# DPDK/grout

Hardware: AMD Instinct MI355X
Metric: Mpps IPv4 forward, 64B pkts, ~1M-route FIB (device-resident), 1/8 GPU (higher is better)
Workload: dtype u8/u32 integer

## Files before the change

grout_amd/csrc/fwd4_kernel.h:

```cpp
#pragma once

#include "../../include/grout_hip.h"

#include <stdint.h>

#define FWD4_STAT_SLOTS 32
#define FWD4_STAT_SHARDS 64
#define FWD4_MAX_ETH_TYPES 16

struct fwd4_edges {
	uint16_t eth_type_be[FWD4_MAX_ETH_TYPES];
	uint8_t eth_type_edge[FWD4_MAX_ETH_TYPES];
	uint8_t n_eth_types;
	uint8_t mode[GR_HIP_IFACE_MODE_COUNT];
	uint8_t in_nh[8];
	uint8_t out_nh[8];
	uint8_t out_iface[8];
	uint8_t iout_type[8];
	uint8_t in6_nh[8];
	uint8_t out6_nh[8];
	uint8_t out6_iface[8];
};

#define FWD4_RX_MAC_OK 0x01
// ... 110 lines not shown
	uint32_t out_stride;
	uint32_t readable;
	uint32_t nhf_lds;
	uint32_t nhf6_lds;
	const uint32_t *top6;
	uint32_t top6_lds;
	uint32_t chunk;
	uint32_t order;
	uint32_t spin_max;
	uint32_t *err;
	uint32_t wg0, wgs;
	uint32_t ptrs;
	uint32_t nat;
};

struct __attribute__((aligned(64))) fwd4_res_desc {
	uint64_t seq;
	uint64_t helper_seq[7];
	struct fwd4_params A;
};

struct fwd4_res_params {
	struct fwd4_res_desc *descs;
	uint64_t *done;
	uint64_t *exited;
	uint32_t *stop;
	uint64_t *wake;
	uint64_t *active;
	const uint32_t *taken;
	uint64_t lifetime;
// ... 14 lines not shown
```

grout_amd/csrc/fwd4_ring.hip:

```cpp
#include "fwd4_chain.h"

#define RING_GLDS_PER_TILE 6
#define RING_SPIN_MAX (1u << 24)
#define RING_NHF_LDS_MAX 2304

template <int WAVES_, int LOADERS_, int STORERS_, int SLOTS_, int AHEAD_>
struct ring_cfg {
	static constexpr uint32_t WAVES = WAVES_, LOADERS = LOADERS_, STORERS = STORERS_;
	static constexpr uint32_t COMPUTE = WAVES_ - LOADERS_ - STORERS_;
	static constexpr uint32_t SLOTS = SLOTS_, AHEAD = AHEAD_;
	static constexpr int VMCNT_AHEAD = RING_GLDS_PER_TILE * (AHEAD_ - 1);
	static_assert(COMPUTE >= 1 && SLOTS_ >= LOADERS_ * AHEAD_ && VMCNT_AHEAD <= 63, "ring geometry");
};

typedef ring_cfg<8, 1, 1, 8, 4> ring_cfg0;
typedef ring_cfg<8, 2, 1, 8, 3> ring_cfg1;
typedef ring_cfg<16, 2, 2, 16, 4> ring_cfg2;
typedef ring_cfg<12, 2, 1, 12, 4> ring_cfg3;
typedef ring_cfg<8, 1, 1, 8, 6> ring_cfg4;
typedef ring_cfg<16, 2, 2, 16, 6> ring_cfg5;
typedef ring_cfg<16, 3, 1, 20, 4> ring_cfg6;
typedef ring_cfg<16, 4, 2, 24, 3> ring_cfg7;
typedef ring_cfg<16, 2, 2, 16, 8> ring_cfg8;
typedef ring_cfg<14, 1, 1, 8, 8> ring_cfg9;
typedef ring_cfg<14, 2, 2, 8, 4> ring_cfg10;
typedef ring_cfg<12, 1, 1, 8, 8> ring_cfg11;
#define RING_NCFG 15

template <class C, bool PTRS>
struct ring_lds {
	uint8_t lines[C::SLOTS][64 * 64];
	u2v meta[C::SLOTS][64];
	uint64_t ptrs[PTRS ? C::SLOTS : 1][64];
	uint32_t ready[C::SLOTS], done[C::SLOTS], free_[C::SLOTS];
	uint32_t abort;
	uint32_t spin_max;
};

template <int N>
__device__ __forceinline__ void wait_vmcnt() {
	asm volatile("s_waitcnt vmcnt(%0)" ::"n"(N) : "memory");
}

__device__ __forceinline__ uint32_t lds_addr(const void *p) {
	return (uint32_t)(uintptr_t)(const __attribute__((address_space(3))) void *)p;
}

template <bool NT>
__device__ __forceinline__ void glds16(const void *gsrc, uint32_t lds_base) {
	uint32_t keep;
	if (NT)
// ... 11 lines not shown
template <bool NT>
__device__ __forceinline__ void glds4(const void *gsrc, uint32_t lds_base) {
	uint32_t keep;
	if (NT)
		asm volatile("s_mov_b32 %0, m0\n\ts_mov_b32 m0, %2\n\ts_nop 0\n\tglobal_load_lds_dword %1, off nt\n\ts_mov_b32 m0, %0"
			     : "=&s"(keep)
			     : "v"(gsrc), "s"(lds_base)
			     : "memory");
	else
		asm volatile("s_mov_b32 %0, m0\n\ts_mov_b32 m0, %2\n\ts_nop 0\n\tglobal_load_lds_dword %1, off\n\ts_mov_b32 m0, %0"
			     : "=&s"(keep)
			     : "v"(gsrc), "s"(lds_base)
			     : "memory");
}

__device__ __forceinline__ uint32_t flag_get(const uint32_t *f) {
	return __hip_atomic_load(f, __ATOMIC_RELAXED, __HIP_MEMORY_SCOPE_WORKGROUP);
}

__device__ __forceinline__ void flag_set(uint32_t *f, uint32_t v) {
	compiler_fence();
	__hip_atomic_store(f, v, __ATOMIC_RELAXED, __HIP_MEMORY_SCOPE_WORKGROUP);
}

template <class L_t>
__device__ __forceinline__ bool flag_wait(L_t &L, const uint32_t *f, uint32_t want) {
	const uint32_t lim = L.spin_max;
	for (uint32_t spin = 0;; spin++) {
		if ((int32_t)(flag_get(f) - want) >= 0)
			return true;
		if (flag_get(&L.abort))
			return false;
		if (spin >= lim) {
			flag_set(&L.abort, 1);
			return false;
		}
		__builtin_amdgcn_s_sleep(1);
	}
}

__device__ __forceinline__ uint32_t wg_id(const fwd4_params &A) {
	return A.wgs ? A.wg0 : blockIdx.x;
}
__device__ __forceinline__ uint32_t wg_count(const fwd4_params &A) {
	return A.wgs ? A.wgs : gridDim.x;
}

__device__ __forceinline__ uint32_t tile_of(const fwd4_params &A, uint32_t k) {
	const uint32_t b = wg_id(A), G = wg_count(A);
	if (A.order == 2) {
		const uint32_t x = b & 7, l = b >> 3, per = G >> 3;
		return x * A.chunk + l + k * per;
	}
	if (A.order == 3) {
		const uint32_t j = k / A.chunk;
// ... 18 lines not shown
	if (A.chunk)
		return b * A.chunk < n_tiles ? min(A.chunk, n_tiles - b * A.chunk) : 0;
	return b < n_tiles ? (n_tiles - 1 - b) / G + 1 : 0;
}

__device__ __forceinline__ uint64_t load_ptr(const fwd4_params &A, uint32_t t, uint32_t lane) {
	const uint32_t i = min(t * 64 + lane, A.n - 1);
	return gld(reinterpret_cast<const uint64_t *>(A.in) + i);
}

__device__ __forceinline__ uint64_t shfl64(uint64_t v, uint32_t src) {
	const uint32_t lo = __shfl((uint32_t)v, (int)src, 64), hi = __shfl((uint32_t)(v >> 32), (int)src, 64);
	return ((uint64_t)hi << 32) | lo;
}

template <class C, bool NT, bool PTRS, class LT>
__device__ void ring_loader(const fwd4_params &A, LT &L, uint32_t n_local, uint32_t j, uint32_t lane) {
	const uint32_t prow = lane >> 2;
	const uint32_t pchunk = (lane & 3) ^ ((lane >> 4) & 3);
	uint32_t pub = j;
	bool ok = true;
	uint64_t pnext = 0;
	if (PTRS && j < n_local)
		pnext = load_ptr(A, tile_of(A, j), lane);
	for (uint32_t k = j; k < n_local && ok; k += C::LOADERS) {
		const uint32_t s = k % C::SLOTS;
		if (k >= C::SLOTS && (int32_t)(flag_get(&L.free_[s]) - (k - C::SLOTS + 1)) < 0) {
			wait_vmcnt<0>();
			for (; pub < k; pub += C::LOADERS)
				flag_set(&L.ready[pub % C::SLOTS], pub + 1);
			ok = flag_wait(L, &L.free_[s], k - C::SLOTS + 1);
			if (!ok)
				break;
		}
		const uint32_t t = tile_of(A, k);
		const uint32_t base = t * 64, last = min(64u, A.n - base) - 1;
		uint64_t pk = 0;
		if (PTRS) {
			pk = pnext;
			if (k + C::LOADERS < n_local)
				pnext = load_ptr(A, tile_of(A, k + C::LOADERS), lane);
			if (k == j)
				wait_vmcnt<0>();
			else
				wait_vmcnt<RING_GLDS_PER_TILE>();
			L.ptrs[s][lane] = pk;
		}
		const uint32_t lb = lds_addr(L.lines[s]);
#pragma unroll
		for (uint32_t q = 0; q < 4; q++) {
			const uint32_t r = min(q * 16 + prow, last);
			const uint8_t *src = PTRS ? reinterpret_cast<const uint8_t *>(shfl64(pk, r))
						  : A.in + (size_t)(base + r) * A.in_stride;
			glds16<NT>(src + pchunk * 16, lb + q * 1024);
		}
		const uint32_t mb = lds_addr(L.meta[s]);
		const uint8_t *msrc = reinterpret_cast<const uint8_t *>(A.meta + base);
#pragma unroll
		for (uint32_t q = 0; q < 2; q++) {
			const uint32_t pkt = min(q * 32 + (lane >> 1), last);
			glds4<NT>(msrc + pkt * 8 + (lane & 1) * 4, mb + q * 256);
		}
		if (k - pub == (C::AHEAD - 1) * C::LOADERS) {
			wait_vmcnt<C::VMCNT_AHEAD>();
			flag_set(&L.ready[pub % C::SLOTS], pub + 1);
			pub += C::LOADERS;
		}
	}
	wait_vmcnt<0>();
	if (ok)
		for (; pub < n_local; pub += C::LOADERS)
			flag_set(&L.ready[pub % C::SLOTS], pub + 1);
}

template <class C, bool NT, bool PTRS, class LT>
__device__ void ring_storer(const fwd4_params &A, LT &L, uint32_t n_local, uint32_t j, uint32_t lane) {
	const uint32_t prow = lane >> 2, part = lane & 3;
	const uint32_t pslot = (part ^ ((lane >> 4) & 3)) << 4;
	const bool prefix = A.out_stride == GR_HIP_PREFIX;
	for (uint32_t k = j; k < n_local; k += C::STORERS) {
		const uint32_t s = k % C::SLOTS;
		if (!flag_wait(L, &L.done[s], k + 1))
			break;
		const uint32_t t = tile_of(A, k);
		const uint32_t base = t * 64, cnt = min(64u, A.n - base);
		u4v o[4];
#pragma unroll
		for (uint32_t q = 0; q < 4; q++)
			o[q] = *reinterpret_cast<const u4v *>(&L.lines[s][(q * 16 + prow) * 64 + pslot]);
		const u2v v = L.meta[s][lane];
		uint8_t *dst[4];
#pragma unroll
		for (uint32_t q = 0; q < 4; q++) {
			const uint32_t r = q * 16 + prow;
			dst[q] = PTRS && A.out == nullptr ? reinterpret_cast<uint8_t *>(L.ptrs[s][r])
							  : A.out + (size_t)(base + r) * A.out_stride;
		}
		asm volatile("s_waitcnt lgkmcnt(0)" ::: "memory");
		flag_set(&L.free_[s], k + 1);
// ... 29 lines not shown
		(const __attribute__((address_space(4))) uint32_t *)(((uint64_t)bhi << 32) | blo);
	uint32_t sv[SG];
#pragma unroll
	for (int i = 0; i < SG; i++)
		sv[i] = base[(uint32_t)__builtin_amdgcn_readlane(idx, i)];
	uint32_t v = 0, w = 0;
	if (want && lane >= (uint32_t)SG)
		v = gld(rx.tbl24 + idx);
#pragma unroll
	for (int i = 0; i < SG; i++)
		asm volatile("v_writelane_b32 %0, %1, %2" : "+v"(w) : "s"(sv[i]), "i"(i));
	ent = lane < (uint32_t)SG ? w : v;
	return want;
}

template <class C, bool STATS, bool PTRS, int SG = 0, class LT>
__device__ void ring_compute(const fwd4_params &A, const kctx &P, LT &L, stat_slot *slots,
			     const uint4 *nhf_lds, uint32_t n_local, uint32_t c, uint32_t lane) {
	for (uint32_t k = c; k < n_local; k += C::COMPUTE) {
		const uint32_t s = k % C::SLOTS;
		if (!flag_wait(L, &L.ready[s], k + 1))
			break;
		const uint32_t t = tile_of(A, k);
		const uint32_t base = t * 64, cnt = min(64u, A.n - base);
		const bool live = lane < cnt;
		uint8_t *R = L.lines[s];
		gr_hip_pkt_meta m = {0, 0, 0, 0};
		if (live) {
			const u2v pm = L.meta[s][lane];
			m.iface = pm.x & 0xffff;
			m.vlan_ck = pm.x >> 16;
			m.pkt_len = pm.y & 0xffff;
			m.rss = pm.y >> 16;
		}
		const uint32_t if0 = __builtin_amdgcn_readfirstlane(m.iface);
		rxv rx;
		if (__ballot(live && m.iface != if0) == 0)
			rx = load_rx_scalar(P, if0);
// ... 63 lines not shown
			c0.z = 0;
			lds_put(R, lane, 0, c0);
		}
		L.meta[s][lane] = u2v{r.edge | (r.domain << 8) | (r.iface << 16), r.nh};
		flag_set(&L.done[s], k + 1);
		if (STATS) {
			const uint32_t len = m.pkt_len;
			wave_count(slots, P, r.rx_if ? r.rx_if + 1 : 0, len);
			wave_count(slots, P, r.rx_par ? r.rx_par + 1 : 0, len);
			wave_count(slots, P, r.tx_if ? (r.tx_if | 0x10000u) + 1 : 0, len);
			wave_count(slots, P, r.tx_par ? (r.tx_par | 0x10000u) + 1 : 0, len);
		}
	}
}

#ifdef RING_TRACE
#define RING_TRACE_MAX 4096
__device__ uint64_t ring_trace[2 * RING_TRACE_MAX];
extern "C" int gr_fwd4_ring_trace(uint64_t *out, uint32_t n) {
	if (n > 2 * RING_TRACE_MAX)
		n = 2 * RING_TRACE_MAX;
	return hipMemcpyFromSymbol(out, HIP_SYMBOL(ring_trace), n * sizeof(uint64_t)) == hipSuccess ? 0 : -5;
}
#endif

template <class C, bool STATS, bool NT, bool PTRS = false, int SG = 0>
__global__ void __launch_bounds__(C::WAVES * 64) gr_fwd4_ring(const fwd4_params A) {
#ifdef RING_TRACE
	if (threadIdx.x == 0 && blockIdx.x < RING_TRACE_MAX)
		ring_trace[2 * blockIdx.x] = __builtin_amdgcn_s_memrealtime();
#endif
	__shared__ __attribute__((aligned(16))) ring_lds<C, PTRS> L;
	__shared__ stat_slot slots[FWD4_STAT_SLOTS];
	__shared__ fwd4_edges edges;
	extern __shared__ __attribute__((aligned(16))) uint4 nhf_lds[];
	const uint32_t tid = threadIdx.x, lane = tid & 63;
	const uint32_t wv = __builtin_amdgcn_readfirstlane(tid >> 6);
	const fwd4_tables *T = A.T;

	{
		const uint4 *src = reinterpret_cast<const uint4 *>(T->nhf) + 1;
		for (uint32_t i = tid; i < A.nhf_lds; i += C::WAVES * 64)
			nhf_lds[i] = gld4(src + i);
		const uint4 *src6 = reinterpret_cast<const uint4 *>(T->nhf6) + 1;
		for (uint32_t i = tid; i < A.nhf6_lds; i += C::WAVES * 64)
			nhf_lds[A.nhf_lds + i] = gld4(src6 + i);
		uint32_t *top6 = reinterpret_cast<uint32_t *>(nhf_lds + A.nhf_lds + A.nhf6_lds);
		for (uint32_t i = tid; i < A.top6_lds; i += C::WAVES * 64)
			top6[i] = gld(A.top6 + FWD4_TOP6_BASE + i);
	}
	for (uint32_t i = tid; i < sizeof(fwd4_edges); i += C::WAVES * 64)
		reinterpret_cast<uint8_t *>(&edges)[i] = reinterpret_cast<const uint8_t *>(&T->edges)[i];
	if (tid < C::SLOTS) {
		L.ready[tid] = 0;
		L.done[tid] = 0;
		L.free_[tid] = 0;
	}
	if (tid == 0) {
		L.abort = 0;
		L.spin_max = A.spin_max ? A.spin_max : RING_SPIN_MAX;
	}
	if (STATS && tid < FWD4_STAT_SLOTS) {
		slots[tid].key = 0;
		slots[tid].pkts = 0;
		slots[tid].bytes = 0;
	}
	__syncthreads();

	const uint32_t n_local = local_tiles(A);
	if (wv < C::LOADERS) {
		ring_loader<C, NT, PTRS>(A, L, n_local, wv, lane);
	} else if (wv < C::LOADERS + C::STORERS) {
		ring_storer<C, NT, PTRS>(A, L, n_local, wv - C::LOADERS, lane);
	} else {
		kctx P = make_kctx(A, &edges);
		P.nhf6_lds = (const __attribute__((address_space(3))) u4v *)(nhf_lds + A.nhf_lds);
		P.nhf6_n = A.nhf6_lds;
		P.top6 = A.top6;
		P.top6_lds = (const __attribute__((address_space(3))) uint32_t *)(nhf_lds + A.nhf_lds + A.nhf6_lds);
		P.top6_n = A.top6_lds;
		ring_compute<C, STATS, PTRS, SG>(A, P, L, slots, nhf_lds, n_local, wv - C::LOADERS - C::STORERS, lane);
	}

	__syncthreads();
	if (tid == 0 && L.abort && A.err != nullptr)
		__hip_atomic_store(A.err, 1u, __ATOMIC_RELAXED, __HIP_MEMORY_SCOPE_SYSTEM);
	if (STATS) {
		if (tid < FWD4_STAT_SLOTS && slots[tid].key != 0) {
			const uint32_t key = slots[tid].key - 1;
			shard_add(A.stats, T->max_ifaces, key >> 16, key & 0xffff, slots[tid].pkts, slots[tid].bytes);
		}
	}
#ifdef RING_TRACE
	__syncthreads();
	if (tid == 0 && blockIdx.x < RING_TRACE_MAX) {
		ring_trace[2 * blockIdx.x + 1] = __builtin_amdgcn_s_memrealtime();
	}
#endif
}

typedef ring_cfg2 ring_cfg_res;

__device__ __forceinline__ uint64_t sys_load64(const uint64_t *p) {
	return __hip_atomic_load(p, __ATOMIC_ACQUIRE, __HIP_MEMORY_SCOPE_SYSTEM);
}

__global__ void __launch_bounds__(ring_cfg_res::WAVES * 64) gr_fwd4_resident(const fwd4_res_params R) {
	typedef ring_cfg_res C;
	__shared__ __attribute__((aligned(16))) ring_lds<C, true> L;
	__shared__ __attribute__((aligned(16))) fwd4_params A;
	__shared__ fwd4_edges edges;
	__shared__ uint64_t seq_s;
	__shared__ uint32_t go;
	const uint32_t tid = threadIdx.x, lane = tid & 63;
	const uint32_t wv = __builtin_amdgcn_readfirstlane(tid >> 6);
	uint64_t *done = R.done + (size_t)blockIdx.x * R.stride;
	const fwd4_res_desc *ring = R.descs + (size_t)blockIdx.x * R.ndesc;
	uint64_t idle_since = __builtin_amdgcn_s_memrealtime();
	if (tid == 0) {
		seq_s = sys_load64(done) + 1;
		go = __hip_atomic_load(R.taken + blockIdx.x, __ATOMIC_RELAXED, __HIP_MEMORY_SCOPE_SYSTEM);
	}
	__syncthreads();
	if (go == 0) {
		if (tid == 0)
			__hip_atomic_store(R.exited + (size_t)blockIdx.x * R.stride, R.launch_id, __ATOMIC_RELEASE,
					   __HIP_MEMORY_SCOPE_SYSTEM);
		return;
	}
	const bool helper = go == 2;
// ... 56 lines not shown
			reinterpret_cast<uint8_t *>(&edges)[i] = reinterpret_cast<const uint8_t *>(&A.T->edges)[i];
		if (tid < C::SLOTS) {
			L.ready[tid] = 0;
			L.done[tid] = 0;
			L.free_[tid] = 0;
		}
		if (tid == 0) {
			L.abort = 0;
			L.spin_max = A.spin_max ? A.spin_max : RING_SPIN_MAX;
		}
		__syncthreads();
		const uint32_t n_local = local_tiles(A);
		const bool ptrs = A.ptrs != 0;
		if (wv < C::LOADERS) {
			if (ptrs)
				ring_loader<C, false, true>(A, L, n_local, wv, lane);
			else
				ring_loader<C, false, false>(A, L, n_local, wv, lane);
		} else if (wv < C::LOADERS + C::STORERS) {
			if (ptrs)
				ring_storer<C, false, true>(A, L, n_local, wv - C::LOADERS, lane);
			else
				ring_storer<C, false, false>(A, L, n_local, wv - C::LOADERS, lane);
		} else {
			const kctx P = make_kctx(A, &edges);
			if (ptrs)
				ring_compute<C, false, true>(A, P, L, nullptr, nullptr, n_local, wv - C::LOADERS - C::STORERS, lane);
			else
				ring_compute<C, false, false>(A, P, L, nullptr, nullptr, n_local, wv - C::LOADERS - C::STORERS, lane);
		}
		wait_vmcnt<0>();
		__syncthreads();
		if (tid == 0) {
			if (L.abort && A.err != nullptr)
				__hip_atomic_store(A.err, 1u, __ATOMIC_RELAXED, __HIP_MEMORY_SCOPE_SYSTEM);
			__hip_atomic_store(done, seq_s, __ATOMIC_RELEASE, __HIP_MEMORY_SCOPE_SYSTEM);
			seq_s++;
			idle_since = __builtin_amdgcn_s_memrealtime();
			__hip_atomic_store(R.active, idle_since, __ATOMIC_RELAXED, __HIP_MEMORY_SCOPE_AGENT);
		}
		__syncthreads();
	}
	if (tid == 0)
		__hip_atomic_store(R.exited + (size_t)blockIdx.x * R.stride, R.launch_id, __ATOMIC_RELEASE,
// ... 24 lines not shown
	const unsigned long long v = reset ? __hip_atomic_exchange(p, 0ull, __ATOMIC_RELAXED, __HIP_MEMORY_SCOPE_AGENT)
					   : __hip_atomic_fetch_add(p, 0ull, __ATOMIC_RELAXED, __HIP_MEMORY_SCOPE_AGENT);
	__hip_atomic_store(out + i, v, __ATOMIC_RELAXED, __HIP_MEMORY_SCOPE_SYSTEM);
}

extern "C" hipError_t gr_stats_collect_launch(void *d, void *out, uint32_t w, uint32_t pitch, uint32_t rows, int reset,
					      hipStream_t s) {
	const uint32_t n = w * 4 * rows;
	if (n == 0)
		return hipSuccess;
	hipLaunchKernelGGL(gr_stats_collect, dim3((n + 255) / 256), dim3(256), 0, s, static_cast<unsigned long long *>(d),
			   static_cast<unsigned long long *>(out), w, pitch, rows, reset);
	return hipGetLastError();
}

typedef void (*fwd4_rfn)(const fwd4_params);
struct ring_entry {
	fwd4_rfn fn[4];
	uint32_t threads;
};
#define RING_ENTRY_SG(C, SG) {{gr_fwd4_ring<C, false, false, false, SG>, gr_fwd4_ring<C, true, false, false, SG>, \
			 gr_fwd4_ring<C, false, true, false, SG>, gr_fwd4_ring<C, true, true, false, SG>}, C::WAVES * 64}
#define RING_ENTRY(C) RING_ENTRY_SG(C, 0)
static const ring_entry ring_kernels[RING_NCFG] = {
	RING_ENTRY(ring_cfg0), RING_ENTRY(ring_cfg1), RING_ENTRY(ring_cfg2),
	RING_ENTRY(ring_cfg3), RING_ENTRY(ring_cfg4), RING_ENTRY(ring_cfg5),
	RING_ENTRY(ring_cfg6), RING_ENTRY(ring_cfg7), RING_ENTRY(ring_cfg8),
	RING_ENTRY(ring_cfg9), RING_ENTRY(ring_cfg10), RING_ENTRY(ring_cfg11),
	RING_ENTRY_SG(ring_cfg2, 16), RING_ENTRY_SG(ring_cfg2, 32), RING_ENTRY_SG(ring_cfg2, 64),
};

#define RING_PTRS_CFG 2
typedef ring_cfg2 ring_cfg_ptrs;
static const ring_entry ring_ptrs_kernel = {
	{gr_fwd4_ring<ring_cfg_ptrs, false, false, true>, gr_fwd4_ring<ring_cfg_ptrs, true, false, true>,
	 gr_fwd4_ring<ring_cfg_ptrs, false, true, true>, gr_fwd4_ring<ring_cfg_ptrs, true, true, true>},
	ring_cfg_ptrs::WAVES * 64};

extern "C" hipError_t gr_fwd4_ring_launch(const fwd4_params *A, uint32_t grid, hipStream_t s, int variant, int cfg) {
	const ring_entry &e = (variant & FWD4_V_PTRS) ? ring_ptrs_kernel : ring_kernels[(unsigned)cfg % RING_NCFG];
	const size_t lds = (A->nhf_lds + A->nhf6_lds) * sizeof(fwd4_nhf) + A->top6_lds * sizeof(uint32_t);
	hipLaunchKernelGGL(e.fn[variant & 3], dim3(grid), dim3(e.threads), lds, s, *A);
	return hipGetLastError();
}

extern "C" uint32_t gr_fwd4_ring_nhf_max(void) {
	return RING_NHF_LDS_MAX;
}

extern "C" int gr_fwd4_ring_ncfg(void) {
	return RING_NCFG;
}

extern "C" int gr_fwd4_ring_occupancy(int variant, int cfg, uint32_t nhf_lds) {
	const ring_entry &e = (variant & FWD4_V_PTRS) ? ring_ptrs_kernel : ring_kernels[(unsigned)cfg % RING_NCFG];
	int b = 0;
	if (hipOccupancyMaxActiveBlocksPerMultiprocessor(&b, e.fn[variant & 3], (int)e.threads, nhf_lds * sizeof(fwd4_nhf))
// ... 7 lines not shown
```

grout_amd/csrc/gr_hip.cpp:

```cpp
#include <hip/hip_runtime.h>

#include "fib4.h"
#include "fib6.h"
#include "fwd4_kernel.h"
#include "gr_node_priv.h"

#include <algorithm>
#include <atomic>
#include <errno.h>
#include <map>
#include <mutex>
#include <shared_mutex>
#include <new>
#include <stdio.h>
#include <time.h>
#include <unistd.h>
#include <stdlib.h>
#include <string.h>
#include <vector>

extern "C" hipError_t gr_fwd4_ring_launch(const fwd4_params *A, uint32_t grid, hipStream_t s, int variant, int cfg);
extern "C" int gr_fwd4_ring_occupancy(int variant, int cfg, uint32_t nhf_lds);
extern "C" hipError_t gr_fwd4_resident_launch(const fwd4_res_params *R, uint32_t rings, hipStream_t s);
extern "C" hipError_t gr_stats_collect_launch(void *d, void *out, uint32_t w, uint32_t pitch, uint32_t rows, int reset,
					      hipStream_t s);
extern "C" uint32_t gr_fwd4_ring_nhf_max(void);
extern "C" int gr_fwd4_resident_occupancy(void);
extern "C" int gr_fwd4_ring_ncfg(void);
#define RING_WG_PER_CU 2


#define HCK(expr)                                                                                  \
	do {                                                                                       \
		hipError_t e__ = (expr);                                                           \
		if (e__ != hipSuccess) {                                                           \
			(void)hipGetLastError();                                                   \
			if (getenv("GR_HIP_TRACE_ERRORS"))                                         \
				fprintf(stderr, "gr_hip: %s:%d: %s: %s\n", __FILE__, __LINE__, #expr, \
					hipGetErrorString(e__));                                   \
			return e__ == hipErrorOutOfMemory ? -ENOMEM : -EIO;                        \
		}                                                                                  \
	} while (0)

namespace {
// ... 130 lines not shown
	bool own_stream;
	hipEvent_t ev0[N_TIMED], ev1[N_TIMED];
	uint64_t n_launch;
	uint64_t n_submit;
	bool always_timed;
	hipEvent_t quiesce;
	hipEvent_t retire;
	uint64_t seen_serial;
	hipEvent_t sync_ev;
	gr_hip_iface_stats *d_stats;
	host_slot hs[HOST_SLOTS];
	node_slot nw[GR_HIP_NODE_DEPTH];
	uint32_t nw_head, nw_count;
	uint8_t *d_pad;
	uint32_t *h_err, *d_err;
	std::vector<gr_hip_iface_stats> node_if;
	std::vector<gr_hip_iface_stats> kern_seen;
	gr_hip_iface_stats *snap = nullptr;
	void *snap_d = nullptr;
	uint32_t snap_cap = 0, snap_w = 0;
	gr_hip_iface_stats *rd = nullptr;
	void *rd_d = nullptr;
	uint32_t rd_cap = 0;
	hipEvent_t snap_ev = nullptr;
	bool snap_pending = false;
	uint64_t node_counted = 0, snap_counted = 0;
	uint8_t *pg_lines = nullptr, *pg_out = nullptr;
	gr_hip_pkt_meta *pg_meta = nullptr;
	gr_hip_verdict *pg_v = nullptr;
	uint32_t pg_cap = 0;
// ... 91 lines not shown
	uint32_t *d_snat_vals = nullptr;
	uint32_t snat_cap = 0;
	fwd4_edges edges;
	fwd4_tables *d_tables[2];
	std::vector<gr_hip_queue *> queues;
	int nt;
	int stats_on;
	int wg_per_cu;
	int fib_fmt;
	int ring_cfg;
	int host_direct;
	int node_ptrs;
	uint32_t stage_min_tiles;
	int tile_order;
	uint32_t tile_run;
	int alloc_contig;
	uint32_t spin_max;
	std::atomic<int> fail_appends{0};
	int untimed;
	uint32_t time_every;
	int stats_copy;
	int sync_check;
	std::atomic<int> host_path_last{-1};
	std::vector<host_range> hregs;
	int res_on;
	uint32_t res_rings;
	uint32_t res_w;
	uint32_t res_ms;
	uint32_t res_nap;
	uint32_t res_tiles;
// ... 472 lines not shown
		goto fail;
	if (hipMemsetAsync(c->d_adj, 0, sizeof(fwd4_adj) * ((size_t)max_nexthops + 1), c->ctl) != hipSuccess
	    || hipMemsetAsync(c->d_nhf, 0, sizeof(fwd4_nhf) * ((size_t)max_nexthops + 1), c->ctl) != hipSuccess
	    || hipMemsetAsync(c->d_nhf6, 0, sizeof(fwd4_nhf) * ((size_t)max_nexthops + 1), c->ctl) != hipSuccess
	    || hipMemsetAsync(c->d_adj6, 0, sizeof(fwd4_adj6) * ((size_t)max_nexthops + 1), c->ctl) != hipSuccess)
		goto fail;
	c->nt = FWD4_V_NT;
	c->stats_on = 1;
	c->wg_per_cu = 0;
	c->fib_fmt = FIB_FMT_24_W2;
	c->ring_cfg = 2;
	c->host_direct = 1;
	c->node_ptrs = 0;
	c->tile_order = 0;
	c->tile_run = 16;
	c->stage_min_tiles = 4;
	c->res_on = 0;
	c->res_rings = 256;
	c->res_w = 8;
	c->res_ms = 50;
	c->res_nap = 16;
	c->res_tiles = 8;
	c->spin_max = 0;
	c->untimed = 0;
	c->time_every = 1;
	c->alloc_contig = 1;
	for (int v = 0; v < 8; v++)
		c->occ_ring[v] = gr_fwd4_ring_occupancy(v, 0, 0);
	c->occ_n = 0;
	ret = -EIO;
// ... 1063 lines not shown
		hipEventCreate(&q->ev1[i]);
	}
	hipEventCreateWithFlags(&q->quiesce, hipEventDisableTiming);
	hipEventCreateWithFlags(&q->retire, hipEventDisableTiming);
	hipEventCreateWithFlags(&q->sync_ev, hipEventDisableTiming);
	for (node_slot &w : q->nw)
		hipEventCreateWithFlags(&w.done, hipEventDisableTiming);
	hipEventRecord(q->retire, q->s);
	if (hipHostMalloc(reinterpret_cast<void **>(&q->h_err), sizeof(uint32_t), hipHostMallocMapped) == hipSuccess) {
		*q->h_err = 0;
		if (hipHostGetDevicePointer(reinterpret_cast<void **>(&q->d_err), q->h_err, 0) != hipSuccess) {
			hipHostFree(q->h_err);
			q->h_err = q->d_err = nullptr;
		}
	}
	(void)hipGetLastError();
	size_t sb = sizeof(gr_hip_iface_stats) * FWD4_STAT_SHARDS * c->max_ifaces;
	if (hipMalloc(&q->d_stats, sb) != hipSuccess || hipMemsetAsync(q->d_stats, 0, sb, q->s) != hipSuccess) {
		(void)hipGetLastError();
		q->d_stats = nullptr;
	}
	try {
		q->node_if.assign(c->max_ifaces, gr_hip_iface_stats{0, 0, 0, 0});
		q->kern_seen.assign(c->max_ifaces, gr_hip_iface_stats{0, 0, 0, 0});
	} catch (...) {
		return -ENOMEM;
	}
	c->queues.push_back(q);
	*out = q;
	return 0;
// ... 36 lines not shown
		if (h.s)
			hipStreamDestroy(h.s);
		hipFree(h.in);
		hipFree(h.out);
		hipFree(h.meta);
		hipFree(h.v);
	}
	for (uint32_t i = 0; i < N_TIMED; i++) {
		hipEventDestroy(q->ev0[i]);
		hipEventDestroy(q->ev1[i]);
	}
	hipEventDestroy(q->quiesce);
	hipEventDestroy(q->retire);
	hipEventDestroy(q->sync_ev);
	hipFree(q->d_stats);
	if (q->snap_ev != nullptr)
		hipEventDestroy(q->snap_ev);
	hipHostFree(q->snap);
	hipHostFree(q->rd);
	hipHostFree(q->h_err);
	hipHostFree(q->pg_lines);
	hipHostFree(q->pg_out);
	hipHostFree(q->pg_meta);
	hipHostFree(q->pg_v);
	for (node_slot &w : q->nw) {
		hipEventDestroy(w.done);
		if (q->dead)
			continue;
		hipHostFree(w.lines);
		hipHostFree(w.out);
// ... 106 lines not shown
	uint32_t grid = (uint32_t)c->n_cu * per_cu;
	if (grid > tiles)
		grid = tiles;
	A.err = q->d_err;
	A.spin_max = c->spin_max;
	A.order = c->tile_order;
	A.chunk = 0;
	if (c->tile_order == 1)
		A.chunk = (tiles + grid - 1) / grid;
	if (c->tile_order == 2 && grid % 8 == 0)
		A.chunk = (tiles + 7) / 8;
	else if (c->tile_order == 2)
		A.order = 0;
	if (c->tile_order == 3)
		A.chunk = c->tile_run;
	if (timed && !q->always_timed) {
		const uint64_t k = q->n_submit++;
		timed = !c->untimed && (c->time_every <= 1 || k % c->time_every == 0);
	}
	if (timed)
		HCK(hipEventRecord(q->ev0[slot], s));
	HCK(gr_fwd4_ring_launch(&A, grid, s, variant, c->ring_cfg));
	if (timed) {
		HCK(hipEventRecord(q->ev1[slot], s));
		q->n_launch++;
	}
	return 0;
}

#define RES_NDESC 8
static_assert(GR_HIP_NODE_DEPTH < RES_NDESC, "a ring's batches in flight fit its descriptors");
#define RES_STRIDE 8
#define RES_TILES_PER_WG 8
#define RES_LEAVE_NS (500ull * 1000000ull)

static uint64_t res_word(const uint64_t *w, int ring) {
	return __atomic_load_n(w + (size_t)ring * RES_STRIDE, __ATOMIC_ACQUIRE);
// ... 455 lines not shown
		c->res_ms = (uint32_t)value;
	} else if (strcmp(key, "resident_launches") == 0) {
		return (int)c->res_launch;
	} else if (strcmp(key, "resident_ring_count") == 0) {
		return (int)c->res_rings;
	} else if (strcmp(key, "resident_busy") == 0) {
		return (int)c->res_busy.load();
	} else if (strcmp(key, "stage_min_tiles") == 0) {
		if (value < 0)
			return -EINVAL;
		c->stage_min_tiles = (uint32_t)value;
	} else if (strcmp(key, "tile_run") == 0) {
		if (value < 1 || value > 4096)
			return -EINVAL;
		c->tile_run = (uint32_t)value;
	} else if (strcmp(key, "host_direct") == 0) {
		c->host_direct = value != 0;
	} else if (strcmp(key, "fib_format_of") == 0) {
		if (value <= 0 || (uint32_t)value >= c->max_ifaces || c->vrfs[value].rib == nullptr
		    || !c->vrfs[value].uploaded())
			return -ENONET;
		return c->vrfs[value].pub().fmt;
	} else if (strcmp(key, "fib16") == 0) {
		c->fib_fmt = value ? FIB_FMT_16_8_8 : FIB_FMT_24;
	} else if (strcmp(key, "ring") == 0) {
		if (value < 0 || value >= gr_fwd4_ring_ncfg())
			return -EINVAL;
		c->ring_cfg = value;
	} else if (strncmp(key, "commit_us_", 10) == 0) {
		const char *k = key + 10;
// ... 1131 lines not shown
```

Before: 38620.

## Add dynamic tile claiming via global atomic counter for ring kernel tail balancing

The ring kernel now assigns most tiles statically, then leaves a tail share (default 32/256) that workgroups claim in runs of 8 tiles through a global atomic counter. The loader wave issues the atomic ahead of need and publishes run bases in LDS, and compute and storer waves read the tile id from LDS instead of recomputing it. The goal is to remove load imbalance and straggler workgroups at the end of each launch. The cost is an atomic round trip per run, extra LDS flags and end-of-stream handling, and a double-buffered counter that block 0 resets for the next launch.

```diff
diff --git a/grout_amd/csrc/fwd4_kernel.h b/grout_amd/csrc/fwd4_kernel.h
--- a/grout_amd/csrc/fwd4_kernel.h
+++ b/grout_amd/csrc/fwd4_kernel.h
@@ -148,6 +148,39 @@
 	uint32_t nat;
 };
 
+#define FWD4_CLAIM_SHARE_MAX 256u
+
+#ifdef __HIPCC__
+#define FWD4_HD __host__ __device__
+#else
+#define FWD4_HD
+#endif
+
+static inline FWD4_HD uint32_t fwd4_claim_n_static(uint32_t n_tiles, uint32_t G, uint32_t share) {
+	if (share > FWD4_CLAIM_SHARE_MAX)
+		share = FWD4_CLAIM_SHARE_MAX;
+	const uint32_t want = (uint32_t)(((uint64_t)n_tiles * share + FWD4_CLAIM_SHARE_MAX - 1) / FWD4_CLAIM_SHARE_MAX);
+	return G ? (n_tiles - want) / G : 0;
+}
+
+static inline FWD4_HD uint64_t fwd4_claim_run_base(uint32_t n_static, uint32_t G, uint32_t run, uint32_t g) {
+	return (uint64_t)n_static * G + (uint64_t)g * run;
+}
+
+static inline FWD4_HD uint32_t fwd4_claim_run_len(uint32_t n_tiles, uint64_t base, uint32_t run) {
+	if (base >= n_tiles)
+		return 0;
+	const uint32_t left = n_tiles - (uint32_t)base;
+	return left < run ? left : run;
+}
+
+struct fwd4_claim {
+	uint32_t *ctr;
+	uint32_t *ctr_next;
+	uint32_t n_static;
+	uint32_t run;
+};
+
 struct __attribute__((aligned(64))) fwd4_res_desc {
 	uint64_t seq;
 	uint64_t helper_seq[7];
diff --git a/grout_amd/csrc/fwd4_ring.hip b/grout_amd/csrc/fwd4_ring.hip
--- a/grout_amd/csrc/fwd4_ring.hip
+++ b/grout_amd/csrc/fwd4_ring.hip
@@ -3,6 +3,7 @@
 #define RING_GLDS_PER_TILE 6
 #define RING_SPIN_MAX (1u << 24)
 #define RING_NHF_LDS_MAX 2304
+#define RING_CLAIM_NR 64
 
 template <int WAVES_, int LOADERS_, int STORERS_, int SLOTS_, int AHEAD_>
 struct ring_cfg {
@@ -11,6 +12,7 @@
 	static constexpr uint32_t SLOTS = SLOTS_, AHEAD = AHEAD_;
 	static constexpr int VMCNT_AHEAD = RING_GLDS_PER_TILE * (AHEAD_ - 1);
 	static_assert(COMPUTE >= 1 && SLOTS_ >= LOADERS_ * AHEAD_ && VMCNT_AHEAD <= 63, "ring geometry");
+	static_assert(SLOTS_ + (AHEAD_ + 1) * LOADERS_ + 2 <= RING_CLAIM_NR, "claimed runs in LDS");
 };
 
 typedef ring_cfg<8, 1, 1, 8, 4> ring_cfg0;
@@ -35,6 +37,10 @@
 	uint32_t ready[C::SLOTS], done[C::SLOTS], free_[C::SLOTS];
 	uint32_t abort;
 	uint32_t spin_max;
+	uint32_t tile[C::SLOTS];
+	uint32_t run_base[RING_CLAIM_NR];
+	uint32_t runs;
+	uint32_t end;
 };
 
 template <int N>
@@ -76,6 +82,16 @@
 			     : "memory");
 }
 
+#ifdef RING_TRACE
+#define RING_TRACE_MAX 4096
+__device__ uint64_t ring_trace[4 * RING_TRACE_MAX];
+extern "C" int gr_fwd4_ring_trace(uint64_t *out, uint32_t n) {
+	if (n > 4 * RING_TRACE_MAX)
+		n = 4 * RING_TRACE_MAX;
+	return hipMemcpyFromSymbol(out, HIP_SYMBOL(ring_trace), n * sizeof(uint64_t)) == hipSuccess ? 0 : -5;
+}
+#endif
+
 __device__ __forceinline__ uint32_t flag_get(const uint32_t *f) {
 	return __hip_atomic_load(f, __ATOMIC_RELAXED, __HIP_MEMORY_SCOPE_WORKGROUP);
 }
@@ -101,6 +117,92 @@
 	}
 }
 
+template <class L_t>
+__device__ __forceinline__ int flag_wait_k(L_t &L, const uint32_t *f, uint32_t want, uint32_t k) {
+	const uint32_t lim = L.spin_max;
+	for (uint32_t spin = 0;; spin++) {
+		if ((int32_t)(flag_get(f) - want) >= 0)
+			return 1;
+		if (flag_get(&L.abort))
+			return 0;
+		const uint32_t e = flag_get(&L.end);
+		if (e != 0 && k >= e - 1)
+			return 2;
+		if (spin >= lim) {
+			flag_set(&L.abort, 1);
+			return 0;
+		}
+		__builtin_amdgcn_s_sleep(1);
+	}
+}
+
+__device__ __forceinline__ uint32_t claim_box() {
+	uint32_t box;
+	asm volatile("v_mov_b32 %0, 0" : "=v"(box));
+	return box;
+}
+
+__device__ __forceinline__ void claim_issue(uint32_t *ctr, uint32_t box) {
+	uint64_t keep;
+	asm volatile("s_mov_b64 %0, exec\n\ts_mov_b64 exec, 1\n\tglobal_atomic_add %1, %2, %3, off sc0\n\ts_mov_b64 exec, %0"
+		     : "=&s"(keep)
+		     : "v"(box), "v"(ctr), "v"(1u)
+		     : "memory");
+}
+
+template <int N>
+__device__ __forceinline__ uint32_t claim_read(uint32_t box) {
+	uint32_t g;
+	asm volatile("s_waitcnt vmcnt(%2)\n\tv_readfirstlane_b32 %0, %1" : "=s"(g) : "v"(box), "n"(N) : "memory");
+	return g;
+}
+
+struct claim_state {
+	uint32_t n_claim;
+	uint32_t since;
+	bool pending, ended;
+};
+
+template <int N, class LT>
+__device__ __forceinline__ void claim_take(const fwd4_params &A, const fwd4_claim &Q, LT &L, claim_state &cs, uint32_t box,
+					   uint32_t &n_known) {
+	const uint32_t g = claim_read<N>(box);
+	const uint32_t n_tiles = (A.n + 63) >> 6;
+	const uint64_t base = fwd4_claim_run_base(Q.n_static, gridDim.x, Q.run, g);
+	const uint32_t len = fwd4_claim_run_len(n_tiles, base, Q.run);
+	cs.pending = false;
+	if (len != 0)
+		L.run_base[cs.n_claim % RING_CLAIM_NR] = (uint32_t)base;
+	n_known += len;
+	if (len < Q.run) {
+		cs.ended = true;
+		flag_set(&L.end, n_known + 1);
+	}
+	cs.n_claim++;
+	flag_set(&L.runs, cs.n_claim);
+}
+
+template <class C, class LT>
+__device__ __forceinline__ void claim_step(const fwd4_params &A, const fwd4_claim &Q, LT &L, claim_state &cs, uint32_t box,
+					   uint32_t &n_known, uint32_t k) {
+	while (!cs.ended) {
+		if (cs.pending) {
+			if (cs.since < C::AHEAD - 1) {
+				if (k < n_known)
+					break;
+				wait_vmcnt<0>();
+			}
+			claim_take<C::VMCNT_AHEAD>(A, Q, L, cs, box, n_known);
+		} else {
+			if (k + C::AHEAD * C::LOADERS < n_known)
+				break;
+			claim_issue(Q.ctr, box);
+			cs.pending = true;
+			cs.since = 0;
+		}
+	}
+}
+
 __device__ __forceinline__ uint32_t wg_id(const fwd4_params &A) {
 	return A.wgs ? A.wg0 : blockIdx.x;
 }
@@ -149,8 +251,9 @@
 	return ((uint64_t)hi << 32) | lo;
 }
 
-template <class C, bool NT, bool PTRS, class LT>
-__device__ void ring_loader(const fwd4_params &A, LT &L, uint32_t n_local, uint32_t j, uint32_t lane) {
+template <class C, bool NT, bool PTRS, bool CLAIM, class LT>
+__device__ void ring_loader(const fwd4_params &A, const fwd4_claim &Q, LT &L, uint32_t n_local, uint32_t j, uint32_t lane) {
+	static_assert(!(CLAIM && PTRS), "frame-pointer launches keep the static order");
 	const uint32_t prow = lane >> 2;
 	const uint32_t pchunk = (lane & 3) ^ ((lane >> 4) & 3);
 	uint32_t pub = j;
@@ -158,7 +261,34 @@
 	uint64_t pnext = 0;
 	if (PTRS && j < n_local)
 		pnext = load_ptr(A, tile_of(A, j), lane);
-	for (uint32_t k = j; k < n_local && ok; k += C::LOADERS) {
+	const bool dyn = CLAIM && Q.ctr != nullptr;
+	claim_state cs = {0, 0, false, !dyn};
+	const uint32_t box = CLAIM ? claim_box() : 0;
+	uint32_t k = j;
+	for (; ok; k += C::LOADERS) {
+		uint32_t t = 0;
+		if (CLAIM && dyn && j == 0)
+			claim_step<C>(A, Q, L, cs, box, n_local, k);
+		if (CLAIM && dyn && k >= Q.n_static) {
+			const uint32_t i = (k - Q.n_static) / Q.run;
+			if (j != 0 && (int32_t)(flag_get(&L.runs) - (i + 1)) < 0) {
+				wait_vmcnt<0>();
+				for (; pub < k; pub += C::LOADERS)
+					flag_set(&L.ready[pub % C::SLOTS], pub + 1);
+				if (flag_wait_k(L, &L.runs, i + 1, k) == 0) {
+					ok = false;
+					break;
+				}
+			}
+			const uint32_t e = flag_get(&L.end);
+			if (e != 0 && k >= e - 1)
+				break;
+			t = __builtin_amdgcn_readfirstlane(L.run_base[i % RING_CLAIM_NR]) + (k - Q.n_static) % Q.run;
+		} else {
+			if (k >= n_local && cs.ended)
+				break;
+			t = tile_of(A, k);
+		}
 		const uint32_t s = k % C::SLOTS;
 		if (k >= C::SLOTS && (int32_t)(flag_get(&L.free_[s]) - (k - C::SLOTS + 1)) < 0) {
 			wait_vmcnt<0>();
@@ -168,8 +298,13 @@
 			if (!ok)
 				break;
 		}
-		const uint32_t t = tile_of(A, k);
 		const uint32_t base = t * 64, last = min(64u, A.n - base) - 1;
+		if (CLAIM)
+			L.tile[s] = t;
+#ifdef RING_TRACE
+		if (k == 0 && lane == 0 && blockIdx.x < RING_TRACE_MAX)
+			ring_trace[4 * blockIdx.x + 2] = __builtin_amdgcn_s_memrealtime();
+#endif
 		uint64_t pk = 0;
 		if (PTRS) {
 			pk = pnext;
@@ -196,6 +331,7 @@
 			const uint32_t pkt = min(q * 32 + (lane >> 1), last);
 			glds4<NT>(msrc + pkt * 8 + (lane & 1) * 4, mb + q * 256);
 		}
+		cs.since++;
 		if (k - pub == (C::AHEAD - 1) * C::LOADERS) {
 			wait_vmcnt<C::VMCNT_AHEAD>();
 			flag_set(&L.ready[pub % C::SLOTS], pub + 1);
@@ -204,20 +340,24 @@
 	}
 	wait_vmcnt<0>();
 	if (ok)
-		for (; pub < n_local; pub += C::LOADERS)
+		for (; pub < k; pub += C::LOADERS)
 			flag_set(&L.ready[pub % C::SLOTS], pub + 1);
-}
-
-template <class C, bool NT, bool PTRS, class LT>
+#ifdef RING_TRACE
+	if (CLAIM && j == 0 && lane == 0 && blockIdx.x < RING_TRACE_MAX)
+		ring_trace[4 * blockIdx.x + 3] = cs.n_claim;
+#endif
+}
+
+template <class C, bool NT, bool PTRS, bool CLAIM, class LT>
 __device__ void ring_storer(const fwd4_params &A, LT &L, uint32_t n_local, uint32_t j, uint32_t lane) {
 	const uint32_t prow = lane >> 2, part = lane & 3;
 	const uint32_t pslot = (part ^ ((lane >> 4) & 3)) << 4;
 	const bool prefix = A.out_stride == GR_HIP_PREFIX;
-	for (uint32_t k = j; k < n_local; k += C::STORERS) {
+	for (uint32_t k = j; CLAIM || k < n_local; k += C::STORERS) {
 		const uint32_t s = k % C::SLOTS;
-		if (!flag_wait(L, &L.done[s], k + 1))
+		if (CLAIM ? flag_wait_k(L, &L.done[s], k + 1, k) != 1 : !flag_wait(L, &L.done[s], k + 1))
 			break;
-		const uint32_t t = tile_of(A, k);
+		const uint32_t t = CLAIM ? __builtin_amdgcn_readfirstlane(L.tile[s]) : tile_of(A, k);
 		const uint32_t base = t * 64, cnt = min(64u, A.n - base);
 		u4v o[4];
 #pragma unroll
@@ -277,14 +417,14 @@
 	return want;
 }
 
-template <class C, bool STATS, bool PTRS, int SG = 0, class LT>
+template <class C, bool STATS, bool PTRS, bool CLAIM, int SG = 0, class LT>
 __device__ void ring_compute(const fwd4_params &A, const kctx &P, LT &L, stat_slot *slots,
 			     const uint4 *nhf_lds, uint32_t n_local, uint32_t c, uint32_t lane) {
-	for (uint32_t k = c; k < n_local; k += C::COMPUTE) {
+	for (uint32_t k = c; CLAIM || k < n_local; k += C::COMPUTE) {
 		const uint32_t s = k % C::SLOTS;
-		if (!flag_wait(L, &L.ready[s], k + 1))
+		if (CLAIM ? flag_wait_k(L, &L.ready[s], k + 1, k) != 1 : !flag_wait(L, &L.ready[s], k + 1))
 			break;
-		const uint32_t t = tile_of(A, k);
+		const uint32_t t = CLAIM ? __builtin_amdgcn_readfirstlane(L.tile[s]) : tile_of(A, k);
 		const uint32_t base = t * 64, cnt = min(64u, A.n - base);
 		const bool live = lane < cnt;
 		uint8_t *R = L.lines[s];
@@ -378,21 +518,14 @@
 	}
 }
 
+template <class C, bool STATS, bool NT, bool PTRS = false, int SG = 0>
+__global__ void __launch_bounds__(C::WAVES * 64) gr_fwd4_ring(const fwd4_params A, const fwd4_claim Q) {
+	constexpr bool CLAIM = !PTRS;
 #ifdef RING_TRACE
-#define RING_TRACE_MAX 4096
-__device__ uint64_t ring_trace[2 * RING_TRACE_MAX];
-extern "C" int gr_fwd4_ring_trace(uint64_t *out, uint32_t n) {
-	if (n > 2 * RING_TRACE_MAX)
-		n = 2 * RING_TRACE_MAX;
-	return hipMemcpyFromSymbol(out, HIP_SYMBOL(ring_trace), n * sizeof(uint64_t)) == hipSuccess ? 0 : -5;
-}
-#endif
-
-template <class C, bool STATS, bool NT, bool PTRS = false, int SG = 0>
-__global__ void __launch_bounds__(C::WAVES * 64) gr_fwd4_ring(const fwd4_params A) {
-#ifdef RING_TRACE
-	if (threadIdx.x == 0 && blockIdx.x < RING_TRACE_MAX)
-		ring_trace[2 * blockIdx.x] = __builtin_amdgcn_s_memrealtime();
+	if (threadIdx.x == 0 && blockIdx.x < RING_TRACE_MAX) {
+		ring_trace[4 * blockIdx.x] = __builtin_amdgcn_s_memrealtime();
+		ring_trace[4 * blockIdx.x + 3] = 0;
+	}
 #endif
 	__shared__ __attribute__((aligned(16))) ring_lds<C, PTRS> L;
 	__shared__ stat_slot slots[FWD4_STAT_SLOTS];
@@ -420,9 +553,13 @@
 		L.done[tid] = 0;
 		L.free_[tid] = 0;
 	}
+	const bool dyn = CLAIM && Q.ctr != nullptr;
+	const uint32_t n_local = dyn ? Q.n_static : local_tiles(A);
 	if (tid == 0) {
 		L.abort = 0;
 		L.spin_max = A.spin_max ? A.spin_max : RING_SPIN_MAX;
+		L.runs = 0;
+		L.end = dyn ? 0 : n_local + 1;
 	}
 	if (STATS && tid < FWD4_STAT_SLOTS) {
 		slots[tid].key = 0;
@@ -431,11 +568,10 @@
 	}
 	__syncthreads();
 
-	const uint32_t n_local = local_tiles(A);
 	if (wv < C::LOADERS) {
-		ring_loader<C, NT, PTRS>(A, L, n_local, wv, lane);
+		ring_loader<C, NT, PTRS, CLAIM>(A, Q, L, n_local, wv, lane);
 	} else if (wv < C::LOADERS + C::STORERS) {
-		ring_storer<C, NT, PTRS>(A, L, n_local, wv - C::LOADERS, lane);
+		ring_storer<C, NT, PTRS, CLAIM>(A, L, n_local, wv - C::LOADERS, lane);
 	} else {
 		kctx P = make_kctx(A, &edges);
 		P.nhf6_lds = (const __attribute__((address_space(3))) u4v *)(nhf_lds + A.nhf_lds);
@@ -443,12 +579,14 @@
 		P.top6 = A.top6;
 		P.top6_lds = (const __attribute__((address_space(3))) uint32_t *)(nhf_lds + A.nhf_lds + A.nhf6_lds);
 		P.top6_n = A.top6_lds;
-		ring_compute<C, STATS, PTRS, SG>(A, P, L, slots, nhf_lds, n_local, wv - C::LOADERS - C::STORERS, lane);
+		ring_compute<C, STATS, PTRS, CLAIM, SG>(A, P, L, slots, nhf_lds, n_local, wv - C::LOADERS - C::STORERS, lane);
 	}
 
 	__syncthreads();
 	if (tid == 0 && L.abort && A.err != nullptr)
 		__hip_atomic_store(A.err, 1u, __ATOMIC_RELAXED, __HIP_MEMORY_SCOPE_SYSTEM);
+	if (CLAIM && tid == 0 && blockIdx.x == 0 && Q.ctr_next != nullptr)
+		__hip_atomic_store(Q.ctr_next, 0u, __ATOMIC_RELAXED, __HIP_MEMORY_SCOPE_AGENT);
 	if (STATS) {
 		if (tid < FWD4_STAT_SLOTS && slots[tid].key != 0) {
 			const uint32_t key = slots[tid].key - 1;
@@ -457,9 +595,8 @@
 	}
 #ifdef RING_TRACE
 	__syncthreads();
-	if (tid == 0 && blockIdx.x < RING_TRACE_MAX) {
-		ring_trace[2 * blockIdx.x + 1] = __builtin_amdgcn_s_memrealtime();
-	}
+	if (tid == 0 && blockIdx.x < RING_TRACE_MAX)
+		ring_trace[4 * blockIdx.x + 1] = __builtin_amdgcn_s_memrealtime();
 #endif
 }
 
@@ -478,6 +615,7 @@
 	__shared__ uint32_t go;
 	const uint32_t tid = threadIdx.x, lane = tid & 63;
 	const uint32_t wv = __builtin_amdgcn_readfirstlane(tid >> 6);
+	const fwd4_claim Q0 = {nullptr, nullptr, 0, 0};
 	uint64_t *done = R.done + (size_t)blockIdx.x * R.stride;
 	const fwd4_res_desc *ring = R.descs + (size_t)blockIdx.x * R.ndesc;
 	uint64_t idle_since = __builtin_amdgcn_s_memrealtime();
@@ -564,20 +702,20 @@
 		const bool ptrs = A.ptrs != 0;
 		if (wv < C::LOADERS) {
 			if (ptrs)
-				ring_loader<C, false, true>(A, L, n_local, wv, lane);
+				ring_loader<C, false, true, false>(A, Q0, L, n_local, wv, lane);
 			else
-				ring_loader<C, false, false>(A, L, n_local, wv, lane);
+				ring_loader<C, false, false, false>(A, Q0, L, n_local, wv, lane);
 		} else if (wv < C::LOADERS + C::STORERS) {
 			if (ptrs)
-				ring_storer<C, false, true>(A, L, n_local, wv - C::LOADERS, lane);
+				ring_storer<C, false, true, false>(A, L, n_local, wv - C::LOADERS, lane);
 			else
-				ring_storer<C, false, false>(A, L, n_local, wv - C::LOADERS, lane);
+				ring_storer<C, false, false, false>(A, L, n_local, wv - C::LOADERS, lane);
 		} else {
 			const kctx P = make_kctx(A, &edges);
 			if (ptrs)
-				ring_compute<C, false, true>(A, P, L, nullptr, nullptr, n_local, wv - C::LOADERS - C::STORERS, lane);
+				ring_compute<C, false, true, false>(A, P, L, nullptr, nullptr, n_local, wv - C::LOADERS - C::STORERS, lane);
 			else
-				ring_compute<C, false, false>(A, P, L, nullptr, nullptr, n_local, wv - C::LOADERS - C::STORERS, lane);
+				ring_compute<C, false, false, false>(A, P, L, nullptr, nullptr, n_local, wv - C::LOADERS - C::STORERS, lane);
 		}
 		wait_vmcnt<0>();
 		__syncthreads();
@@ -632,7 +770,7 @@
 	return hipGetLastError();
 }
 
-typedef void (*fwd4_rfn)(const fwd4_params);
+typedef void (*fwd4_rfn)(const fwd4_params, const fwd4_claim);
 struct ring_entry {
 	fwd4_rfn fn[4];
 	uint32_t threads;
@@ -655,10 +793,11 @@
 	 gr_fwd4_ring<ring_cfg_ptrs, false, true, true>, gr_fwd4_ring<ring_cfg_ptrs, true, true, true>},
 	ring_cfg_ptrs::WAVES * 64};
 
-extern "C" hipError_t gr_fwd4_ring_launch(const fwd4_params *A, uint32_t grid, hipStream_t s, int variant, int cfg) {
+extern "C" hipError_t gr_fwd4_ring_launch(const fwd4_params *A, const fwd4_claim *Q, uint32_t grid, hipStream_t s, int variant,
+					  int cfg) {
 	const ring_entry &e = (variant & FWD4_V_PTRS) ? ring_ptrs_kernel : ring_kernels[(unsigned)cfg % RING_NCFG];
 	const size_t lds = (A->nhf_lds + A->nhf6_lds) * sizeof(fwd4_nhf) + A->top6_lds * sizeof(uint32_t);
-	hipLaunchKernelGGL(e.fn[variant & 3], dim3(grid), dim3(e.threads), lds, s, *A);
+	hipLaunchKernelGGL(e.fn[variant & 3], dim3(grid), dim3(e.threads), lds, s, *A, *Q);
 	return hipGetLastError();
 }
 
diff --git a/grout_amd/csrc/gr_hip.cpp b/grout_amd/csrc/gr_hip.cpp
--- a/grout_amd/csrc/gr_hip.cpp
+++ b/grout_amd/csrc/gr_hip.cpp
@@ -19,7 +19,8 @@
 #include <string.h>
 #include <vector>
 
-extern "C" hipError_t gr_fwd4_ring_launch(const fwd4_params *A, uint32_t grid, hipStream_t s, int variant, int cfg);
+extern "C" hipError_t gr_fwd4_ring_launch(const fwd4_params *A, const fwd4_claim *Q, uint32_t grid, hipStream_t s, int variant,
+						  int cfg);
 extern "C" int gr_fwd4_ring_occupancy(int variant, int cfg, uint32_t nhf_lds);
 extern "C" hipError_t gr_fwd4_resident_launch(const fwd4_res_params *R, uint32_t rings, hipStream_t s);
 extern "C" hipError_t gr_stats_collect_launch(void *d, void *out, uint32_t w, uint32_t pitch, uint32_t rows, int reset,
@@ -28,6 +29,32 @@
 extern "C" int gr_fwd4_resident_occupancy(void);
 extern "C" int gr_fwd4_ring_ncfg(void);
 #define RING_WG_PER_CU 2
+#define CLAIM_SHARE_DEFAULT 32
+#define CLAIM_RUN_DEFAULT 8
+#define CLAIM_MIN_TILES_DEFAULT 4096
+#define CLAIM_WORD_STRIDE 32
+
+extern "C" uint32_t gr_fwd4_claim_n_static(uint32_t n_tiles, uint32_t grid, uint32_t share) {
+	return fwd4_claim_n_static(n_tiles, grid, share);
+}
+extern "C" uint32_t gr_fwd4_claim_run(uint32_t n_tiles, uint32_t grid, uint32_t n_static, uint32_t run, uint32_t g,
+				      uint64_t *base) {
+	const uint64_t b = fwd4_claim_run_base(n_static, grid, run, g);
+	if (base != nullptr)
+		*base = b;
+	return fwd4_claim_run_len(n_tiles, b, run);
+}
+extern "C" uint32_t gr_fwd4_claim_runs(uint32_t n_tiles, uint32_t grid, uint32_t n_static, uint32_t run, uint64_t *base,
+				       uint32_t *len, uint32_t max) {
+	uint32_t first_empty = max;
+	for (uint32_t g = 0; g < max; g++) {
+		base[g] = fwd4_claim_run_base(n_static, grid, run, g);
+		len[g] = fwd4_claim_run_len(n_tiles, base[g], run);
+		if (len[g] == 0 && first_empty == max)
+			first_empty = g;
+	}
+	return first_empty;
+}
 
 
 #define HCK(expr)                                                                                  \
@@ -188,6 +215,8 @@
 	uint32_t nw_head, nw_count;
 	uint8_t *d_pad;
 	uint32_t *h_err, *d_err;
+	uint32_t *d_claim = nullptr;
+	uint32_t claim_i = 0;
 	std::vector<gr_hip_iface_stats> node_if;
 	std::vector<gr_hip_iface_stats> kern_seen;
 	gr_hip_iface_stats *snap = nullptr;
@@ -309,6 +338,7 @@
 	uint32_t stage_min_tiles;
 	int tile_order;
 	uint32_t tile_run;
+	uint32_t claim_share, claim_run, claim_min_tiles;
 	int alloc_contig;
 	uint32_t spin_max;
 	std::atomic<int> fail_appends{0};
@@ -811,6 +841,9 @@
 	c->node_ptrs = 0;
 	c->tile_order = 0;
 	c->tile_run = 16;
+	c->claim_share = CLAIM_SHARE_DEFAULT;
+	c->claim_run = CLAIM_RUN_DEFAULT;
+	c->claim_min_tiles = CLAIM_MIN_TILES_DEFAULT;
 	c->stage_min_tiles = 4;
 	c->res_on = 0;
 	c->res_rings = 256;
@@ -1904,6 +1937,11 @@
 			q->h_err = q->d_err = nullptr;
 		}
 	}
+	if (hipMalloc(reinterpret_cast<void **>(&q->d_claim), 2 * CLAIM_WORD_STRIDE * sizeof(uint32_t)) != hipSuccess
+	    || hipMemsetAsync(q->d_claim, 0, 2 * CLAIM_WORD_STRIDE * sizeof(uint32_t), q->s) != hipSuccess) {
+		hipFree(q->d_claim);
+		q->d_claim = nullptr;
+	}
 	(void)hipGetLastError();
 	size_t sb = sizeof(gr_hip_iface_stats) * FWD4_STAT_SHARDS * c->max_ifaces;
 	if (hipMalloc(&q->d_stats, sb) != hipSuccess || hipMemsetAsync(q->d_stats, 0, sb, q->s) != hipSuccess) {
@@ -1970,6 +2008,7 @@
 	hipEventDestroy(q->retire);
 	hipEventDestroy(q->sync_ev);
 	hipFree(q->d_stats);
+	hipFree(q->d_claim);
 	if (q->snap_ev != nullptr)
 		hipEventDestroy(q->snap_ev);
 	hipHostFree(q->snap);
@@ -2106,13 +2145,22 @@
 		A.order = 0;
 	if (c->tile_order == 3)
 		A.chunk = c->tile_run;
+	fwd4_claim Q{};
+	if (A.order == 0 && A.chunk == 0 && c->claim_share > 0 && tiles >= c->claim_min_tiles && s == q->s
+	    && q->d_claim != nullptr && !(variant & FWD4_V_PTRS)) {
+		Q.ctr = q->d_claim + q->claim_i * CLAIM_WORD_STRIDE;
+		Q.ctr_next = q->d_claim + (q->claim_i ^ 1) * CLAIM_WORD_STRIDE;
+		Q.n_static = fwd4_claim_n_static(tiles, grid, c->claim_share);
+		Q.run = c->claim_run;
+		q->claim_i ^= 1;
+	}
 	if (timed && !q->always_timed) {
 		const uint64_t k = q->n_submit++;
 		timed = !c->untimed && (c->time_every <= 1 || k % c->time_every == 0);
 	}
 	if (timed)
 		HCK(hipEventRecord(q->ev0[slot], s));
-	HCK(gr_fwd4_ring_launch(&A, grid, s, variant, c->ring_cfg));
+	HCK(gr_fwd4_ring_launch(&A, &Q, grid, s, variant, c->ring_cfg));
 	if (timed) {
 		HCK(hipEventRecord(q->ev1[slot], s));
 		q->n_launch++;
@@ -2598,6 +2646,18 @@
 		if (value < 1 || value > 4096)
 			return -EINVAL;
 		c->tile_run = (uint32_t)value;
+	} else if (strcmp(key, "claim_share") == 0) {
+		if (value < 0 || value > (int)FWD4_CLAIM_SHARE_MAX)
+			return -EINVAL;
+		c->claim_share = (uint32_t)value;
+	} else if (strcmp(key, "claim_run") == 0) {
+		if (value < 1 || value > (1 << 20))
+			return -EINVAL;
+		c->claim_run = (uint32_t)value;
+	} else if (strcmp(key, "claim_min_tiles") == 0) {
+		if (value < 0)
+			return -EINVAL;
+		c->claim_min_tiles = (uint32_t)value;
 	} else if (strcmp(key, "host_direct") == 0) {
 		c->host_direct = value != 0;
 	} else if (strcmp(key, "fib_format_of") == 0) {
```

Result: faster. 39250, median of 6 (+1.6%).
